# polarlightman/Scoring-rules-for-Gaussian-process-regression-a-new-approach-to-inference

Hardware: AMD Instinct MI355X
Metric: GP fit+predict+CRPS wall-clock (ms) at n=20k full / n=40k FITC; HBM GB/s & MFMA% (higher is better)
Workload: dtype f64; 1 GPU; C3 full GP fit(NLML+LOO-CRPS+LOO-LogS)+predict+score; n=20000, d=8, n_test=5000, kernel=ARD, parallelism=single

## Files before the change

### include/gpscore.h

```cpp
#ifndef GPSCORE_H
#define GPSCORE_H

#include <stdint.h>

#ifdef __cplusplus
extern "C" {
#endif

typedef struct gps_ctx gps_ctx;

enum { GPS_ARD = 0, GPS_RBF = 1 };
enum { GPS_FULL = 0, GPS_LOWER = 1 };

enum {
  GPS_OBJ_NLML = 0,
  GPS_OBJ_LOO_CRPS = 1,
  GPS_OBJ_LOO_LOGS = 2,
  GPS_OBJ_LOGDET = 3,
  GPS_OBJ_QUAD = 4,
  GPS_N_OBJ = 5
};
enum {
  GPS_SC_CRPS = 0, GPS_SC_LOGS = 1, GPS_SC_MSLL = 2, GPS_SC_SMSE = 3,
  GPS_SC_MSE = 4, GPS_SC_COVER = 5, GPS_N_SC = 6
// ... 7 lines not shown
const char* gps_last_error(gps_ctx* ctx);
int gps_ctx_set_stream(gps_ctx* ctx, void* hip_stream);
void* gps_ctx_stream(gps_ctx* ctx);
int gps_ctx_synchronize(gps_ctx* ctx);

enum {
  GPS_OPT_OVERLAP = 0,
  GPS_OPT_GEMM_MAP = 3,
  GPS_OPT_TINY_GEMM = 7,
  GPS_OPT_GRAM_REG = 9,
  GPS_OPT_GRAPH = 10,
  GPS_OPT_PRED_PRE = 11,
  GPS_OPT_DAG = 12,
  GPS_OPT_AR_CHUNKS = 15,
  GPS_OPT_DAG_TILES = 13,
  GPS_OPT_STREAM_K = 18,
  GPS_OPT_DAG_WGS = 19,
  GPS_OPT_DAG_GROUP = 17,
  GPS_OPT_SLAB_XCD = 26,
  GPS_OPT_DAG_ORDER = 25,
  GPS_OPT_FITC_DEP = 27,
  GPS_OPT_DAG_TILES_FULL = 28,
  GPS_OPT_DAG_KBATCH = 29,
};
int gps_ctx_set_option(gps_ctx* ctx, int key, int value);

enum { GPS_STAT_GRAPHS = 0, GPS_STAT_GRAPH_CAP = 1, GPS_STAT_GRAPH_OVERFLOW = 2,
       GPS_STAT_DEVICE_BYTES = 3, GPS_STAT_GRAPH_DROPPED = 4, GPS_STAT_GRAPH_EVICTED = 5,
       GPS_N_STATS = 6 };
int gps_ctx_stats(gps_ctx* ctx, int64_t* out, int cap);

int gps_dag_task_list(int T, int flags, uint32_t* out, int cap);
int gps_dag_task_list_ex(int T, int flags, int kb, int kg, uint32_t* out, int cap);

typedef struct gps_gemm_desc {
  int32_t lay_a, lay_b, epi;
  int32_t M, N, K;
  int64_t lda, ldb, ldc;
  double alpha, beta;
  int32_t tri, tri_off;
  int32_t lower_out, mirror;
  int32_t kend;
  int32_t tile, ksplit, map_mode;
  int32_t use_ws, sk_alone, dep_mode;
  int32_t reserved;
  int64_t ld_out, c_kslice_stride;
} gps_gemm_desc;
enum { GPS_GEMM_PLAN_TILE = 0, GPS_GEMM_PLAN_KSPLIT = 1, GPS_GEMM_PLAN_MAP = 2,
       GPS_GEMM_PLAN_SK_DP = 3, GPS_GEMM_PLAN_SK_WGS = 4, GPS_GEMM_PLAN_SLAB_XCD = 5,
       GPS_GEMM_PLAN_GRID_X = 6, GPS_GEMM_PLAN_GRID_Y = 7, GPS_N_GEMM_PLAN = 8 };
int gps_gemm_diag_check(const gps_gemm_desc* d, int have_c, int have_kscale, int have_w,
                        const int32_t* kr, int have_out0, int have_out1);
int gps_gemm_diag(gps_ctx* ctx, const gps_gemm_desc* d, const double* A, const double* B,
                  double* C, const double* kscale, const double* w, const int32_t* kr,
                  double* out0, double* out1, int32_t* plan);
int64_t gps_gemm_schedule(const gps_gemm_desc* d, const int32_t* kr, int have_kscale, int slots,
// ... 170 lines not shown
```

### scoring-rules-for-gaussian-process-regression-a-new-approach-to-inference_amd/csrc/api.hip

```cpp
#include "api_internal.h"

namespace gpsapi {

thread_local std::string g_err;

int fail(gps_ctx* ctx, int code, const std::string& msg) {
  if (ctx) ctx->err = msg;
  g_err = msg;
  return code;
}

hipError_t sync_ctx_streams(gps_ctx* ctx) {
  for (hipStream_t st : {ctx->stream, ctx->side, ctx->aux[0], ctx->aux[1]})
    if (st) {
      const hipError_t e = hipStreamSynchronize(st);
      if (e != hipSuccess) return e;
    }
  return hipSuccess;
}

hipError_t drop_graphs_in(gps_ctx* ctx, const void* p, size_t bytes) {
  if (!ctx || !p || ctx->pgraphs.empty()) return hipSuccess;
  const uintptr_t lo = (uintptr_t)p, hi = lo + bytes;
  bool synced = false;
// ... 192 lines not shown
  const int64_t np = ctx->fn_pad, mp = ctx->m_pad;
  GemmParams p = gp0();
  p.A = ctx->Knm.d(); p.lda = mp; p.B = Lx + c0 * mp; p.ldb = mp;
  p.M = (int)np; p.N = (int)(c1 - c0); p.K = (int)c1; p.tri = TRI_K_LE_J; p.tri_off = (int)c0;
  p.kend = (int)pad_to(ctx->m, 16);
  p.out0 = ctx->fslab.d() + (c0 / GPS_TILE) * np; p.ld_out = np;
  return gemm(ctx, LAY_N, LAY_T, EPI_ROWSQ, p, st);
}

int fitc_rowsq_dep(gps_ctx* ctx, const double* L, int* sig, int64_t ncols, int mode,
                   hipStream_t st, int64_t nb_dag) {
  const int64_t np = ctx->fn_pad, mp = ctx->m_pad;
  GemmParams p = gp0();
  p.A = ctx->Knm.d(); p.lda = mp; p.B = L; p.ldb = mp;
  p.M = (int)np; p.N = (int)ncols; p.K = (int)ncols; p.tri = TRI_K_LE_J;
  p.kend = (int)pad_to(ctx->m, 16);
  p.out0 = ctx->fslab.d(); p.ld_out = np;
  p.dep_sig = sig; p.dep_q = sig + kSigQueue; p.dep_err = static_cast<int*>(ctx->info.p) + 1;
  p.dep_grid = dag_width(ctx, nb_dag, true); p.dep_mode = mode;
  return gemm(ctx, LAY_N, LAY_T, EPI_ROWSQ, p, st);
}

int dag_list_key(const gps_ctx* ctx, int64_t nb) {
  return (int)(3 * nb + ctx->dag_order) << 8 | dag_kg(ctx, nb) << 4 | dag_kb(ctx, nb);
}
int dag_kb(const gps_ctx* ctx, int64_t nb) {
  if ((ctx->dag_kbatch & 256) && nb <= ctx->dag_tiles) return 1;
  return std::max(1, ctx->dag_kbatch & 15);
}
int dag_kg(const gps_ctx* ctx, int64_t nb) { return dag_kb(ctx, nb) > 1 ? ctx->dag_kbatch >> 4 & 3 : 0; }

bool dag_block(const gps_ctx* ctx, int64_t nb) {
  const int cap = ctx->dag_full && ctx->dag_tiles_full ? ctx->dag_tiles_full : ctx->dag_tiles;
  return ctx->dag && nb >= 2 && nb <= cap;
}

void dag_blocks(const gps_ctx* ctx, int64_t nb, std::vector<int>& sizes, int64_t& cnt) {
  if (nb <= 1) return;
  if (dag_block(ctx, nb)) {
    sizes.push_back((int)nb);
    cnt += dag_cnt_ints((int)nb);
    return;
  }
  dag_blocks(ctx, nb / 2, sizes, cnt);
  dag_blocks(ctx, nb - nb / 2, sizes, cnt);
}

int dag_width(const gps_ctx* ctx, int64_t nb, bool half) {
  const int auto_w = half ? std::max(4, ctx->ncu / 2) : ctx->ncu;
  return (int)std::min<int64_t>(ctx->dag_wgs > 0 ? ctx->dag_wgs : auto_w, std::max<int64_t>(4, 2 * nb * nb));
}

int potrf_inv_rec(gps_ctx* ctx, double* A, int64_t lda, double* Linv, int64_t ldl, double* W,
// ... 144 lines not shown
}


hipError_t zero_factor(gps_ctx* ctx, double* p, int64_t n_pad, hipStream_t s) {
  const hipError_t e = hipMemsetAsync(p, 0, (size_t)n_pad * n_pad * 8, s);
  if (e == hipSuccess) ctx->zeroed[(uintptr_t)p] = n_pad;
  return e;
}
bool factor_zeroed(const gps_ctx* ctx, const double* p, int64_t n_pad) {
  const auto it = ctx->zeroed.find((uintptr_t)p);
  return it != ctx->zeroed.end() && it->second == n_pad;
}

int potrf_inv(gps_ctx* ctx, double* A, int64_t n_pad, double* Linv, double* W, double* logdiag,
              int nreal, double* Lout) {
  if (!factor_zeroed(ctx, Linv, n_pad) || (Lout && !factor_zeroed(ctx, Lout, n_pad)))
    return fail(ctx, -1, "potrf_inv: factor buffer not zeroed for this size (internal contract)");
  std::vector<int> dsizes;
  int64_t dcnt = 0;
  dag_blocks(ctx, n_pad / GPS_TILE, dsizes, dcnt);
  for (int T : dsizes) {
    const int lk = dag_list_key(ctx, T);
    if (ctx->dag_lists.count(lk)) continue;
    const std::vector<uint32_t> tl = dag_task_list(T, ctx->dag_order, true, dag_kb(ctx, T), dag_kg(ctx, T));
    auto& e = ctx->dag_lists[lk];
    HIPCHK(ensure(ctx, e.first, tl.size() * 4));
    HIPCHK(hipMemcpyAsync(e.first.p, tl.data(), tl.size() * 4, hipMemcpyHostToDevice, ctx->stream));
    HIPCHK(hipStreamSynchronize(ctx->stream));
    e.second = (int)tl.size();
  }
  if (dcnt && ctx->dag_cnt.cap < (size_t)dcnt * 4) {
    HIPCHK(hipStreamSynchronize(ctx->stream));
    HIPCHK(ensure(ctx, ctx->dag_cnt, std::max<size_t>((size_t)dcnt * 4, (size_t)1 << 20)));
    HIPCHK(hipMemsetAsync(ctx->dag_cnt.p, 0, ctx->dag_cnt.cap, ctx->stream));
    HIPCHK(hipStreamSynchronize(ctx->stream));
  }
  auto eager = [&]() {
    ctx->sync_used = 0;
    ctx->pre.join = nullptr;
    ctx->dag_cnt_used = 0;
    ctx->fplan = gps_ctx::FactorPlan{};
    return potrf_inv_rec(ctx, A, n_pad, Linv, n_pad, W, (int)(n_pad / GPS_TILE), logdiag,
                         static_cast<int*>(ctx->info.p), 0, nreal, Lout, n_pad, true);
  };
  if (!ctx->graphs || ctx->prof || n_pad <= GPS_TILE) return eager();
  HIPCHK(ensure(ctx, ctx->ws_main, (size_t)kSplitWsDoubles * 8));
  HIPCHK(ensure(ctx, ctx->ws_side, (size_t)kSplitWsDoubles * 8));
  const bool pre = ctx->pre.kind == PRE_FITC_Q;
  std::vector<uintptr_t> key = {
      (uintptr_t)A, (uintptr_t)n_pad, (uintptr_t)Linv, (uintptr_t)W, (uintptr_t)logdiag,
      (uintptr_t)nreal, (uintptr_t)Lout, (uintptr_t)ctx->stream, (uintptr_t)ctx->side,
      (uintptr_t)ctx->overlap, (uintptr_t)ctx->gemm_map,
      (uintptr_t)g_tiny_gemm, (uintptr_t)g_stream_k, (uintptr_t)g_slab_xcd, (uintptr_t)ctx->info.p, (uintptr_t)ctx->ws_main.p,
      (uintptr_t)ctx->ws_side.p, (uintptr_t)pre,
      pre ? (uintptr_t)ctx->pre.n1 : 0, pre ? (uintptr_t)ctx->aux[0] : 0,
      pre ? (uintptr_t)ctx->Knm.p : 0, pre ? (uintptr_t)ctx->fslab.p : 0,
      pre ? (uintptr_t)ctx->fn_pad : 0, pre ? (uintptr_t)ctx->m_pad : 0, pre ? (uintptr_t)ctx->pre.sig : 0,
      (uintptr_t)ctx->dag, (uintptr_t)ctx->dag_tiles,
      (uintptr_t)(ctx->dag_full ? ctx->dag_tiles_full : 0), (uintptr_t)ctx->dag_kbatch, (uintptr_t)ctx->dag_group, (uintptr_t)ctx->dag_wgs, (uintptr_t)ctx->dag_half,
      (uintptr_t)ctx->dag_cnt.p, (uintptr_t)ctx->sk_cnt.p, (uintptr_t)ctx->dag_sig};
  for (int T : dsizes) key.push_back((uintptr_t)ctx->dag_lists[dag_list_key(ctx, T)].first.p);
  for (auto& g : ctx->pgraphs)
    if (g.key == key) {
      g.last_use = ++ctx->graph_tick;
      HIPCHK(hipGraphLaunch(g.exec, ctx->stream));
      ctx->fplan = g.plan;
      ctx->fplan.replayed = 1;
      return 0;
    }
  if (ctx->pgraphs.size() >= kMaxGraphs) {
    size_t lru = 0;
    for (size_t i = 1; i < ctx->pgraphs.size(); ++i)
      if (ctx->pgraphs[i].last_use < ctx->pgraphs[lru].last_use) lru = i;
    HIPCHK(sync_ctx_streams(ctx));
    const hipError_t e = hipGraphExecDestroy(ctx->pgraphs[lru].exec);
    ctx->pgraphs.erase(ctx->pgraphs.begin() + (ptrdiff_t)lru);
    ++ctx->graph_evicted;
    HIPCHK(e);
  }
  const size_t nev = 2 * (size_t)(n_pad / GPS_TILE) + 8;
  while (ctx->sync_ev.size() < nev) {
    hipEvent_t e;
// ... 218 lines not shown
      return 0;
    case GPS_OPT_FITC_DEP: ctx->fitc_dep = value != 0; return 0;
    case GPS_OPT_DAG_ORDER:
      ARGCHK(value >= 0 && value <= 2, "GPS_OPT_DAG_ORDER must be 0, 1 or 2");
      ctx->dag_order = value;
      return 0;
    case GPS_OPT_DAG_GROUP:
      ARGCHK(value >= 2 && value <= 4, "GPS_OPT_DAG_GROUP must be 2, 3 or 4");
      ctx->dag_group = value;
      return 0;
    case GPS_OPT_DAG_TILES:
      ARGCHK(value >= 2 && value <= 64, "GPS_OPT_DAG_TILES must be in 2..64");
      ctx->dag_tiles = value;
      return 0;
    case GPS_OPT_DAG_TILES_FULL:
      ARGCHK(value == 0 || (value >= 2 && value <= 64), "GPS_OPT_DAG_TILES_FULL must be 0 or in 2..64");
      ctx->dag_tiles_full = value;
      return 0;
    case GPS_OPT_DAG_KBATCH:
      ARGCHK(value >= 0 && (value & 15) <= 8 && (value >> 4 & 15) <= 3 && (value >> 9) == 0,
             "GPS_OPT_DAG_KBATCH must be B | g << 4 [| 256] with B in 0..8 and g in 0..3");
      ctx->dag_kbatch = (value & 15) < 2 ? 0 : value;
      return 0;
    default: return fail(ctx, -1, "unknown option");
  }
}

void* gps_ctx_stream(gps_ctx* ctx) { return ctx ? (void*)ctx->stream : nullptr; }

int gps_ctx_synchronize(gps_ctx* ctx) {
  if (int rc = bind(ctx)) return rc;
  HIPCHK(hipStreamSynchronize(ctx->stream));
  return 0;
}

int gps_ctx_stats(gps_ctx* ctx, int64_t* out, int cap) {
  if (int rc = bind(ctx)) return rc;
  ARGCHK(out != nullptr && cap >= 0, "out is NULL or cap < 0");
  size_t bytes = 0;
  for (DBuf* b : ctx_buffers(ctx)) bytes += b->cap;
  int64_t v[GPS_N_STATS];
  v[GPS_STAT_GRAPHS] = (int64_t)ctx->pgraphs.size();
  v[GPS_STAT_GRAPH_CAP] = (int64_t)kMaxGraphs;
  v[GPS_STAT_GRAPH_OVERFLOW] = ctx->graph_overflow;
  v[GPS_STAT_GRAPH_DROPPED] = ctx->graph_dropped;
  v[GPS_STAT_GRAPH_EVICTED] = ctx->graph_evicted;
  v[GPS_STAT_DEVICE_BYTES] = (int64_t)bytes;
  for (int i = 0; i < cap && i < GPS_N_STATS; ++i) out[i] = v[i];
  return GPS_N_STATS;
}

int gps_dag_task_list(int T, int flags, uint32_t* out, int cap) {
  return gps_dag_task_list_ex(T, flags, 1, 0, out, cap);
}

int gps_dag_task_list_ex(int T, int flags, int kb, int kg, uint32_t* out, int cap) {
  if (T < 2 || T > 64 || cap < 0 || (cap > 0 && !out) || (flags & ~13) || kb < 1 || kb > 8 || kg < 0 || kg > 3)
    return fail(nullptr, -1, "bad arguments");
  const std::vector<uint32_t> tl = dag_task_list(T, (flags >> 2 & 3) == 0 ? 1 : (flags >> 2 & 3) == 3 ? 0 : flags >> 2 & 3,
                                                 (flags & 1) != 0, kb, kg);
  for (int i = 0; i < cap && i < (int)tl.size(); ++i) out[i] = tl[i];
  return (int)tl.size();
}

int gps_phase_enable(gps_ctx* ctx, int on) {
  if (int rc = bind(ctx)) return rc;
  ctx->phase = on != 0;
  return 0;
}

int gps_phase_collect(gps_ctx* ctx, char* json_out, int64_t cap) {
  if (int rc = bind(ctx)) return rc;
  HIPCHK(sync_ctx_streams(ctx));
  std::map<std::string, std::pair<int, double>> agg;
  std::vector<std::string> order;
  for (size_t i = 1; i < ctx->ph_marks.size(); ++i) {
    const auto& m = ctx->ph_marks[i];
    if (m.first == "start") continue;
    float ms = 0.f;
    HIPCHK(hipEventElapsedTime(&ms, ctx->ph_ev[ctx->ph_marks[i - 1].second], ctx->ph_ev[m.second]));
    if (!agg.count(m.first)) order.push_back(m.first);
    agg[m.first].first += 1;
    agg[m.first].second += ms;
// ... 244 lines not shown
```

### scoring-rules-for-gaussian-process-regression-a-new-approach-to-inference_amd/csrc/api_internal.h

```cpp
#pragma once
#include <dlfcn.h>
#include <rccl/rccl.h>
#include <stdio.h>
#include <string.h>

#include <chrono>
#include <climits>
#include <cmath>
#include <condition_variable>
#include <map>
#include <memory>
#include <mutex>
#include <string>
#include <vector>

#include "gps_internal.h"
#include "gpscore.h"

using namespace gps;

namespace gpsapi {


struct DBuf {
// ... 60 lines not shown

struct gps_ctx {
  int device = 0;
  hipStream_t stream = nullptr;
  bool own_stream = true;
  hipStream_t side = nullptr;
  hipStream_t aux[2] = {nullptr, nullptr};
  bool overlap = true;
  int gemm_map = 0;
  int ar_chunks = 4;
  std::vector<hipEvent_t> ar_ev;
  int ncu = 0;
  std::vector<hipEvent_t> sync_ev;
  size_t sync_used = 0;
  bool graphs = true;
  bool pred_pre = true;
  bool dag = true;
  int dag_tiles = 20;
  int dag_group = 3;
  int dag_wgs = 0;
  int dag_order = 1;
  int dag_tiles_full = 40;
  int dag_kbatch = 8 | 256;
  bool dag_full = false;
  bool dag_half = false;
  bool fitc_dep = true;
  int* dag_sig = nullptr;
  DBuf dsig;
  std::map<int, std::pair<DBuf, int>> dag_lists;
  std::map<uintptr_t, int64_t> zeroed;
  DBuf dag_cnt;
  DBuf sk_cnt;
  int64_t dag_cnt_used = 0;
  struct PrePass {
    int kind = 0;
    int64_t n1 = 0;
    const double* L = nullptr;
    hipEvent_t join = nullptr;
    int* sig = nullptr;
  } pre;
  struct FactorPlan {
    int leaves = 0, dags = 0;
    int dag_tmin = 0, dag_tmax = 0;
    int gemms = 0, replayed = 0;
  } fplan;
  struct PotrfGraph {
// ... 124 lines not shown

hipError_t sync_ctx_streams(gps_ctx* ctx);
hipError_t drop_graphs_in(gps_ctx* ctx, const void* p, size_t bytes);
void forget_zeroed(gps_ctx* ctx, const void* p, size_t bytes);
hipError_t ensure(gps_ctx* ctx, DBuf& b, size_t bytes);
void release(gps_ctx* ctx, DBuf& b);
int get_event(gps_ctx* c);
int phase_event(gps_ctx* c, hipStream_t st);
void phase_mark(gps_ctx* c, const char* name);
hipEvent_t sync_event(gps_ctx* c);
GemmParams gp0();
const char* gemm_tag(int al, int bl, int epi, const GemmParams& p);
double gemm_flops(const GemmParams& p);
int gemm(gps_ctx* ctx, int al, int bl, int epi, const GemmParams& p, hipStream_t st = nullptr,
         GemmLaunchInfo* info = nullptr);
int gram(gps_ctx* ctx, const char* tag, const double* x, int n, const double* xp, int m, int d,
         const Theta& th, double diag_add, int lower, int pad_identity, double* out, int64_t ldo,
         int M, int N, hipStream_t st = nullptr);
int pred_rows(gps_ctx* ctx, int64_t r0, int64_t r1, const double* w, hipStream_t st);
int fitc_rowsq_cols(gps_ctx* ctx, const double* Lx, int64_t c0, int64_t c1, hipStream_t st);
int fitc_rowsq_dep(gps_ctx* ctx, const double* L, int* sig, int64_t ncols, int mode,
                   hipStream_t st, int64_t nb_dag);
int dag_list_key(const gps_ctx* ctx, int64_t nb);
int dag_kb(const gps_ctx* ctx, int64_t nb);
int dag_kg(const gps_ctx* ctx, int64_t nb);
bool dag_block(const gps_ctx* ctx, int64_t nb);
void dag_blocks(const gps_ctx* ctx, int64_t nb, std::vector<int>& sizes, int64_t& cnt);
int dag_width(const gps_ctx* ctx, int64_t nb, bool half);
int potrf_inv_rec(gps_ctx* ctx, double* A, int64_t lda, double* Linv, int64_t ldl, double* W,
                  int nb, double* logdiag, int* info, int base, int nreal, double* Lout,
                  int64_t ldlo, bool top = false);
size_t potrf_ws_doubles(int64_t n_pad);
int reset_info(gps_ctx* ctx);
hipError_t zero_factor(gps_ctx* ctx, double* p, int64_t n_pad, hipStream_t s);
bool factor_zeroed(const gps_ctx* ctx, const double* p, int64_t n_pad);
int potrf_inv(gps_ctx* ctx, double* A, int64_t n_pad, double* Linv, double* W, double* logdiag,
              int nreal, double* Lout);
int check_info(gps_ctx* ctx);
int set_theta(gps_ctx* ctx, Theta& th, int kind, const double* theta, int n_ell, int d);
int upload(gps_ctx* ctx, DBuf& b, const double* h, int64_t rows, int64_t cols, int64_t rows_pad);
void score_bundle(const double* sums, double nt, double out[GPS_N_SC]);
int bind(gps_ctx* ctx);
bool sharded(const gps_ctx* ctx);
std::vector<DBuf*> ctx_buffers(gps_ctx* ctx);
void leave_local_group(gps_ctx* ctx);
int group_barrier(gps_ctx* ctx, LocalGroup& G, size_t count);
// ... 26 lines not shown
```

### scoring-rules-for-gaussian-process-regression-a-new-approach-to-inference_amd/csrc/gps_internal.h

```cpp
#pragma once

#include <hip/hip_runtime.h>
#include <stdint.h>

#include <string>
#include <vector>

#define GPS_TILE 128
#define GPS_MAX_D 64

namespace gps {

inline int64_t pad_to(int64_t n, int64_t t = GPS_TILE) { return (n + t - 1) / t * t; }

struct GramParams {
  const double* x;
  const double* xp;
  double* out;
  int64_t ldo;
  int n, m;
  int M, N;
  int d;
  double sf2;
  double diag_add;
// ... 282 lines not shown
constexpr int kGemmItemInts = 8;
int64_t gemm_schedule(int alay, int blay, int epi, const GemmParams& p, GemmLaunchInfo& info,
                      int32_t* items, int64_t cap);

hipError_t launch_potrf_leaf(const double* A, int64_t lda, double* Linv, int64_t ldl,
                             double* Lout, int64_t ldlo, double* logdiag, int* info,
                             int base, int n_real_in_block, hipStream_t s);

struct DagParams {
  double* A; int64_t lda;
  double* Linv; int64_t ldl;
  double* Lout; int64_t ldlo;
  double* logdiag; int* info; int base; int nreal;
  int T;
  const uint32_t* tasks; int ntasks;
  int* cnt;
  unsigned long long spin_ticks;
  unsigned long long* trace = nullptr;
  int group = 3;
  int* sig = nullptr;
  int kbatch = 1;
};
hipError_t launch_potrf_dag(const DagParams& p, int nwg, hipStream_t s);
std::vector<uint32_t> dag_task_list(int T, int order = 1, bool fine = true, int kb = 1, int kg = 0);
inline int64_t dag_cnt_ints(int T) { return (16 + 2 * (int64_t)T * T + 63) / 64 * 64; }

hipError_t launch_gemv_lower(const double* L, int64_t ldl, const double* x, double* y,
                             int n_pad, hipStream_t s);
hipError_t launch_gemv_full(const double* M, int64_t ldm, const double* x, double* y,
                            int rows, int cols, hipStream_t s);
hipError_t launch_colred(const double* M, int64_t ldm, int rows, int cols, int lower,
                         const double* w, const double* rowscale, double* s1, double* s2,
                         double* slab, hipStream_t s, int crows = 256);
hipError_t launch_slab_sum(const double* slab, int64_t ld, int nslab, int64_t len,
                           const double* init, double* out, hipStream_t s);
hipError_t launch_sym_slab_sum(const double* slab, int64_t slice_stride, int nslab, int M,
                               const double* base, double* dst, hipStream_t s);

hipError_t launch_sym_pack(const double* slab, int64_t slice_stride, int nslab, int r0, int r1,
                           int M, double* packed, hipStream_t s);
hipError_t launch_sym_unpack(const double* packed, int m, int M, const double* base, int full,
                             double* dst, hipStream_t s);
hipError_t launch_full_loo(const double* y, const double* slab, int nslab, int64_t ld,
                           const double* beta, const double* logdiag, int n, double* alpha,
                           double* dinv, double* mu_loo, double* var_loo, double* obj,
                           double* part, hipStream_t s);
hipError_t launch_surface_point_sums(const double* y, const double* alpha, const double* dinv,
// ... 122 lines not shown
```

### scoring-rules-for-gaussian-process-regression-a-new-approach-to-inference_amd/csrc/kernels_potrf.hip

```cpp
#include <algorithm>
#include <queue>
#include <vector>

#include "gps_internal.h"

namespace gps {

namespace v4 {
typedef double d4 __attribute__((ext_vector_type(4)));
typedef double dv2 __attribute__((ext_vector_type(2)));
constexpr int TS = 17;
constexpr int TSZ = 16 * TS;
constexpr int NT = 36;
__device__ __forceinline__ constexpr int tix(int i, int j) { return i * (i + 1) / 2 + j; }

__device__ __forceinline__ double rl(double v, int lane) {
  const int lo = __builtin_amdgcn_readlane(__double2loint(v), lane);
  const int hi = __builtin_amdgcn_readlane(__double2hiint(v), lane);
  return __hiloint2double(hi, lo);
}
template <bool COH>
__device__ __forceinline__ void st_d(double* p, double v) {
  if constexpr (COH)
    __hip_atomic_store(reinterpret_cast<unsigned long long*>(p),
// ... 466 lines not shown
#pragma unroll
        for (int e = 0; e < 4; ++e)
#pragma unroll
          for (int j = 0; j < 2; ++j)
            cold[i][j][e] = ld64(rc, (uint32_t)(((int64_t)(16 * i + g + 4 * e) * s.ldc + 16 * j + r) * 8));
    }
    if (s.bt) wave_gemm32<true, G>(s.A, s.lda, s.B, s.ldb, s.kb, s.ke, acc);
    else wave_gemm32<false, G>(s.A, s.lda, s.B, s.ldb, s.kb, s.ke, acc);
  }
  __syncthreads();
  if (!s.active) return;
#pragma unroll
  for (int i = 0; i < 2; ++i)
#pragma unroll
    for (int e = 0; e < 4; ++e)
#pragma unroll
      for (int j = 0; j < 2; ++j) {
        double v = s.alpha * acc[i][j][e];
        if (s.beta != 0.0) v = fma(s.beta, cold[i][j][e], v);
        const int64_t row = 16 * i + g + 4 * e, col = 16 * j + r;
        st64(rc, (uint32_t)((row * s.ldc + col) * 8), v);
        if (s.C2) s.C2[row * s.ldc2 + col] = v;
      }
}

__device__ __forceinline__ void wave_gemm16(const double* Ap, int64_t lda, const double* B0,
                                            const double* B1, int64_t ldb, int ke0, int ke1,
                                            d4 (&acc)[2]) {
  const int lane = threadIdx.x & 63, r = lane & 15, g = lane >> 4;
  const __amdgpu_buffer_rsrc_t ra = rsrc(Ap, (uint32_t)(16 * lda * 8));
  const __amdgpu_buffer_rsrc_t rb0 = rsrc(B0, (uint32_t)(16 * ldb * 8));
  const __amdgpu_buffer_rsrc_t rb1 = rsrc(B1 ? B1 : B0, (uint32_t)(16 * ldb * 8));
  const int kmax = ke0 > ke1 ? ke0 : ke1;
  double a[8][4], b0[8][4], b1[8][4];
#pragma unroll
  for (int u = 0; u < 8; ++u) {
    const int k = 16 * u + 4 * g;
    const uint32_t o = (uint32_t)(((int64_t)r * lda + k) * 8), ob = (uint32_t)(((int64_t)r * ldb + k) * 8);
    if (16 * u < kmax) {
      const dv2 x0 = ld128(ra, o), x1 = ld128(ra, o + 16);
      a[u][0] = x0.x; a[u][1] = x0.y; a[u][2] = x1.x; a[u][3] = x1.y;
    }
    if (16 * u < ke0) {
      const dv2 x0 = ld128(rb0, ob), x1 = ld128(rb0, ob + 16);
      b0[u][0] = x0.x; b0[u][1] = x0.y; b0[u][2] = x1.x; b0[u][3] = x1.y;
    }
// ... 187 lines not shown
      f.C2 = nullptr;
      f.ldc2 = 0;
      if (type == 1) {
        const int64_t r0 = R + 16 * part;
        f.A = p.A + r0 * lda + K; f.lda = lda;
        f.B = p.Linv + K * ldl + K; f.ldb = ldl;
        f.C = p.A + r0 * lda + K; f.ldc = lda;
        if (p.Lout) { f.C2 = p.Lout + r0 * p.ldlo + K; f.ldc2 = p.ldlo; }
        f.alpha = 1.0; f.beta = 0.0;
        f.c0 = wave; f.c1 = 7 - wave; f.ke0 = 16 * (wave + 1); f.ke1 = 16 * (8 - wave);
        inc = U / NPF_TRSM;
        out = acnt + ti * T + tk;
      } else {
        const int64_t J = 128 * (int64_t)tj, rb = part >> 1, cb = 4 * (part & 1) + wave;
        f.A = p.A + (R + 16 * rb) * lda + K; f.lda = lda;
        f.B = p.A + J * lda + K; f.ldb = lda;
        f.C = p.A + (R + 16 * rb) * lda + J; f.ldc = lda;
        f.alpha = -1.0; f.beta = 1.0;
        f.c0 = (ti == tj && cb > rb) ? -1 : (int)cb; f.c1 = -1; f.ke0 = 128; f.ke1 = 0;
        inc = U / NPF_UPD;
        out = acnt + ti * T + tj;
      }
      run_fine(f);
    } else {
      inc = U / NP;
      Strip st;
      st.C2 = nullptr;
      st.ldc2 = 0;
      st.active = 1;
      const int64_t R = 128 * (int64_t)ti, q = 32 * part, wv = 32 * wave;
      switch (type) {
        case 1: {
          const int64_t K = 128 * (int64_t)tk;
          st.A = p.A + (R + q) * lda + K; st.lda = lda;
          st.B = p.Linv + (K + wv) * ldl + K; st.ldb = ldl; st.bt = 1;
          st.C = p.A + (R + q) * lda + K + wv; st.ldc = lda;
          if (p.Lout) { st.C2 = p.Lout + (R + q) * p.ldlo + K + wv; st.ldc2 = p.ldlo; }
          st.alpha = 1.0; st.beta = 0.0; st.kb = 0; st.ke = (int)wv + 32;
          out = acnt + ti * T + tk;
          break;
        }
        case 2: {
          const int64_t J = 128 * (int64_t)tj, K = 128 * (int64_t)tk;
          st.A = p.A + (R + q) * lda + K; st.lda = lda;
          st.B = p.A + (J + wv) * lda + K; st.ldb = lda; st.bt = 1;
          st.C = p.A + (R + q) * lda + J + wv; st.ldc = lda;
// ... 49 lines not shown
    }
    __syncthreads();
    const int n = 16 + 2 * T * T;
    for (int i = tid; i < n; i += 256)
      __hip_atomic_store(p.cnt + i, 0, __ATOMIC_RELAXED, __HIP_MEMORY_SCOPE_AGENT);
  }
}
}

hipError_t launch_potrf_dag(const DagParams& p, int nwg, hipStream_t s) {
  if ((p.lda & 1) || (p.ldl & 1) || (p.Lout && (p.ldlo & 1)) || p.T < 1 || p.T > 64 || nwg < 1 ||
      !p.tasks || !p.cnt || p.ntasks < 1 || p.kbatch < 1 || p.kbatch > 8)
    return hipErrorInvalidValue;
  if ((int64_t)128 * p.kbatch * std::max(p.lda, p.ldl) * 8 >= ((int64_t)1 << 31)) return hipErrorInvalidValue;
  auto k = p.trace ? (p.group == 2 ? dag::potrf_dag_kernel<true, 2>
                                    : p.group == 3 ? dag::potrf_dag_kernel<true, 3> : dag::potrf_dag_kernel<true, 4>)
                   : (p.group == 2 ? dag::potrf_dag_kernel<false, 2>
                                    : p.group == 3 ? dag::potrf_dag_kernel<false, 3> : dag::potrf_dag_kernel<false, 4>);
  if (p.group < 2 || p.group > 4) return hipErrorInvalidValue;
  hipLaunchKernelGGL(k, dim3(nwg), dim3(256), 0, s, p);
  return hipGetLastError();
}

double g_dag_weights[7] = {35.0, 6.0, 9.7, 11.7, 11.2, 9.3, 2.5};

std::vector<uint32_t> dag_task_list(int T, int order, bool fine, int kb, int kg) {
  struct Task { int type, i, j, k, len; std::vector<int> deps; double est = 0.0, rank = 0.0; };
  auto is_fine = [&](const Task& t) {
    return fine && ((t.type == 1 && t.i == t.k + 1) || (t.type == 2 && t.i == t.k + 1 && t.j == t.i));
  };
  auto batch_of = [&](int t, int nt, int keep, int& b0, int& b1) {
    const int nbat = kb > 1 ? std::max(0, nt - keep) : 0;
    if (t >= nbat) { b0 = t; b1 = t + 1; return; }
    b0 = t / kb * kb;
    b1 = std::min(b0 + kb, nbat);
  };
  std::vector<Task> tk;
  std::vector<int> leaf(T), xkk(T), trsm(T * T, -1), fin(T * T, -1);
  std::vector<int> upd_last(T * T, -1), updx_last(T * T, -1);
  auto add = [&](int type, int i, int j, int k, int len, std::vector<int> deps) {
    Task t;
    t.type = type; t.i = i; t.j = j; t.k = k; t.len = len;
    for (int d : deps)
      if (d >= 0) t.deps.push_back(d);
    tk.push_back(t);
    return (int)tk.size() - 1;
  };
  for (int k = 0; k < T; ++k) {
    leaf[k] = add(0, k, k, k, 1, {upd_last[k * T + k]});
    xkk[k] = leaf[k];
    for (int i = k + 1; i < T; ++i) trsm[i * T + k] = add(1, i, k, k, 1, {upd_last[i * T + k], xkk[k]});
    for (int j = k + 1; j < T; ++j)
      for (int i = j; i < T; ++i) {
        int b0, b1;
        batch_of(k, j, std::max(kg, fine && i == j ? 1 : 0), b0, b1);
        if (k != b1 - 1) continue;
        std::vector<int> deps = {upd_last[i * T + j]};
        for (int q = b0; q < b1; ++q) { deps.push_back(trsm[i * T + q]); deps.push_back(trsm[j * T + q]); }
        if (b1 - b0 == 1) deps = {trsm[i * T + k], trsm[j * T + k], upd_last[i * T + j]};
        upd_last[i * T + j] = add(2, i, j, b0, b1 - b0, deps);
      }
  }
  auto xfinal = [&](int j, int k) { return j == k ? xkk[k] : fin[j * T + k]; };
  for (int j = 0; j < T; ++j) {
    for (int k = 0; k < j; ++k)
      fin[j * T + k] = add(4, j, k, k, 1, {updx_last[j * T + k], xkk[j]});
    for (int i = j + 1; i < T; ++i)
      for (int k = 0; k <= j; ++k) {
        int b0, b1;
        batch_of(j - k, i - k, kg, b0, b1);
        if (j - k != b1 - 1) continue;
        std::vector<int> deps = {updx_last[i * T + k]};
        for (int q = b0 + k; q < b1 + k; ++q) { deps.push_back(trsm[i * T + q]); deps.push_back(xfinal(q, k)); }
        if (b1 - b0 == 1) deps = {trsm[i * T + j], xfinal(j, k), updx_last[i * T + k]};
        updx_last[i * T + k] = add(3, i, b0 + k, k, b1 - b0, deps);
      }
  }
  const int n = (int)tk.size();
  std::vector<std::vector<int>> succ(n);
  std::vector<int> indeg(n, 0);
  for (int t = 0; t < n; ++t)
    for (int d : tk[t].deps) { succ[d].push_back(t); ++indeg[t]; }
  if (order == 0) {
    auto dur = [&](const Task& t) { return t.type == 0 ? 36.0 : 4.0 * t.len; };
    for (int t = 0; t < n; ++t)
      for (int d : tk[t].deps) tk[t].est = std::max(tk[t].est, tk[d].est + dur(tk[d]) + 3.0);
  } else if (order == 2) {
    auto dur = [&](const Task& t) {
      return t.type == 0 ? 38.0 : is_fine(t) ? 4.0 : 9.0 * t.len;
    };
    for (int t = n - 1; t >= 0; --t) {
      double m = 0.0;
      for (int s2 : succ[t]) m = std::max(m, tk[s2].rank + 1.0);
      tk[t].rank = dur(tk[t]) + m;
      tk[t].est = -tk[t].rank;
    }
  } else {
    const double* w = g_dag_weights;
    auto dur = [&](const Task& t) {
      if (is_fine(t)) return w[1];
      switch (t.type) {
        case 0: return w[0];
        case 1: return w[2];
        case 2: return w[3] * t.len;
        case 3: return w[4] * t.len;
        default: return w[5];
      }
    };
    for (int t = n - 1; t >= 0; --t) {
      double m = 0.0;
      for (int s2 : succ[t]) m = std::max(m, tk[s2].rank + w[6]);
      tk[t].rank = dur(tk[t]) + m;
      tk[t].est = -tk[t].rank;
    }
  }
  std::priority_queue<std::pair<double, int>, std::vector<std::pair<double, int>>,
                      std::greater<std::pair<double, int>>> ready;
  for (int t = 0; t < n; ++t)
    if (!indeg[t]) ready.push({tk[t].est, t});
  std::vector<uint32_t> out;
  while (!ready.empty()) {
    const int t = ready.top().second;
    ready.pop();
    const Task& x = tk[t];
    const bool f = is_fine(x);
    const int parts = x.type == 0 ? 1 : !f ? dag::NP : x.type == 1 ? dag::NPF_TRSM : dag::NPF_UPD;
    for (int q = 0; q < parts; ++q)
      out.push_back((uint32_t)x.type | (uint32_t)q << 3 | (uint32_t)f << 7 | (uint32_t)x.i << 8 |
                    (uint32_t)((x.len - 1) & 3) << 14 | (uint32_t)x.j << 16 |
                    (uint32_t)((x.len - 1) >> 2) << 22 | (uint32_t)x.k << 24);
    for (int s2 : succ[t])
      if (!--indeg[s2]) ready.push({tk[s2].est, s2});
  }
  return out;
}

hipError_t launch_potrf_leaf(const double* A, int64_t lda, double* Linv, int64_t ldl, double* Lout,
                             int64_t ldlo, double* logdiag, int* info, int base, int nreal,
                             hipStream_t s) {
  if ((lda & 1) || (ldl & 1) || (Lout && (ldlo & 1))) return hipErrorInvalidValue;
  hipLaunchKernelGGL(v4::potrf_leaf_v4_kernel, dim3(1), dim3(256), 0, s, A, lda, Linv, ldl, Lout,
                     ldlo, logdiag, info, base, nreal);
  return hipGetLastError();
}

}
```

### scoring-rules-for-gaussian-process-regression-a-new-approach-to-inference_amd/gpscore/_lib.py

```python
from __future__ import annotations

import ctypes
import os

import numpy as np

_HERE = os.path.dirname(os.path.abspath(__file__))
LIB_PATH = os.environ.get("GPSCORE_LIB", os.path.join(_HERE, "libgpscore.so"))
ABI_VERSION = 900
GPS_N_STATS = 6
GPS_COMM_NONE, GPS_COMM_RCCL, GPS_COMM_LOCAL = 0, 1, 2
COMM_KINDS = {GPS_COMM_NONE: "none", GPS_COMM_RCCL: "rccl", GPS_COMM_LOCAL: "local"}

GPS_ARD, GPS_RBF = 0, 1
GPS_FULL, GPS_LOWER = 0, 1
GPS_OPT_OVERLAP, GPS_OPT_GEMM_MAP, GPS_OPT_TINY_GEMM, GPS_OPT_GRAM_REG = 0, 3, 7, 9
GPS_OPT_GRAPH = 10
GPS_OPT_PRED_PRE = 11
GPS_OPT_DAG = 12
GPS_OPT_DAG_TILES = 13
GPS_OPT_DAG_GROUP = 17
GPS_OPT_STREAM_K = 18
GPS_OPT_DAG_WGS = 19
GPS_OPT_DAG_ORDER = 25
GPS_OPT_SLAB_XCD = 26
GPS_OPT_FITC_DEP = 27
GPS_OPT_DAG_TILES_FULL = 28
GPS_OPT_DAG_KBATCH = 29
DAG_TILES_FULL_DEFAULT = 40
DAG_KBATCH_DEFAULT = 8 | 256
GPS_OPT_AR_CHUNKS = 15
OBJ_NAMES = ("nlml", "loo_crps", "loo_logs", "logdet", "quad")
SURFACE_NAMES = ("loo_crps", "insample_crps", "nlml", "loo_logs")
GPS_SURF_LOGS_ADD_NOISE = 1
GPS_BATCH_STALE_NOISE = 1
BATCH_MAX_N, BATCH_MAX_D = 128, 16
BATCH_FITC_MAX_M = 32
BATCH_FITC_TALL_MAX_N = 2048
BATCH_FULL_TALL_MAX_N = 512
SCORE_NAMES = ("test_crps", "test_logs", "test_msll", "test_smse", "test_mse", "test_cover")

_c_int, _c_i64, _c_dbl, _c_vp, _c_cp = (ctypes.c_int, ctypes.c_int64, ctypes.c_double,
                                        ctypes.c_void_p, ctypes.c_char_p)
_P = ctypes.POINTER(ctypes.c_double)

_PI = ctypes.POINTER(ctypes.c_int32)
_PI64 = ctypes.POINTER(ctypes.c_int64)
_PP = ctypes.POINTER(_P)


class GemmDesc(ctypes.Structure):
    _fields_ = [("lay_a", ctypes.c_int32), ("lay_b", ctypes.c_int32), ("epi", ctypes.c_int32),
                ("M", ctypes.c_int32), ("N", ctypes.c_int32), ("K", ctypes.c_int32),
# ... 5 lines not shown
                ("tile", ctypes.c_int32), ("ksplit", ctypes.c_int32), ("map_mode", ctypes.c_int32),
                ("use_ws", ctypes.c_int32), ("sk_alone", ctypes.c_int32),
                ("dep_mode", ctypes.c_int32), ("reserved", ctypes.c_int32),
                ("ld_out", _c_i64), ("c_kslice_stride", _c_i64)]


GEMM_PLAN_NAMES = ("tile", "ksplit", "map_mode", "sk_dp", "sk_wgs", "slab_xcd", "grid_x", "grid_y")
POTRF_PLAN_NAMES = ("n_pad", "leaves", "dags", "dag_tmin", "dag_tmax", "gemms", "replayed",
                    "reserved")

SIGNATURES = {
    "gps_version": (_c_int, []),
    "gps_build_id": (_c_int, [_c_cp, _c_int]),
    "gps_ctx_create": (_c_int, [_c_int, ctypes.POINTER(_c_vp)]),
    "gps_ctx_destroy": (_c_int, [_c_vp]),
    "gps_last_error": (_c_cp, [_c_vp]),
    "gps_ctx_set_stream": (_c_int, [_c_vp, _c_vp]),
    "gps_ctx_stream": (_c_vp, [_c_vp]),
    "gps_ctx_synchronize": (_c_int, [_c_vp]),
    "gps_ctx_set_option": (_c_int, [_c_vp, _c_int, _c_int]),
    "gps_ctx_stats": (_c_int, [_c_vp, _c_vp, _c_int]),
    "gps_dag_task_list": (_c_int, [_c_int, _c_int, _c_vp, _c_int]),
    "gps_dag_task_list_ex": (_c_int, [_c_int, _c_int, _c_int, _c_int, _c_vp, _c_int]),
    "gps_gemm_diag_check": (_c_int, [ctypes.POINTER(GemmDesc), _c_int, _c_int, _c_int, _PI, _c_int,
                                     _c_int]),
    "gps_gemm_schedule": (_c_i64, [ctypes.POINTER(GemmDesc), _PI, _c_int, _c_int, _PI, _PI, _c_i64]),
    "gps_gemm_diag": (_c_int, [_c_vp, ctypes.POINTER(GemmDesc), _P, _P, _P, _P, _P, _PI, _P, _P,
                               _PI]),
    "gps_potrf_diag": (_c_int, [_c_vp, _c_i64, _P, _c_i64, _P, _P, _P, _PI, _PI]),
    "gps_grad_terms_diag": (_c_int, [_c_vp, _c_int, _c_int, _c_i64, _c_i64, _c_i64, _c_dbl, _PP,
                                     _PP]),
    "gps_grad_contract_diag": (_c_int, [_c_vp, _c_i64, _c_int, _P, _P, _c_dbl, _P, _P, _c_i64, _P,
                                        _P, _P, _P]),
    "gps_fitc_contract_diag": (_c_int, [_c_vp, _c_i64, _c_i64, _c_i64, _c_int, _P, _P, _P, _c_dbl,
                                        _c_int, _PP, _PI64, _P, _PP, _P, _PP, _PP, _P, _P]),
    "gps_prof_enable": (_c_int, [_c_vp, _c_int]),
    "gps_prof_collect": (_c_int, [_c_vp, _c_cp, _c_i64]),
    "gps_phase_enable": (_c_int, [_c_vp, _c_int]),
    "gps_phase_collect": (_c_int, [_c_vp, _c_cp, _c_i64]),
    "gps_rccl_info": (_c_int, [ctypes.POINTER(_c_int), _c_cp, _c_int]),
    "gps_gram": (_c_int, [_c_vp, _c_int, _P, _c_i64, _P, _c_i64, _c_int, _c_dbl, _P, _c_int,
                          _c_dbl, _c_int, _P]),
    "gps_potrf": (_c_int, [_c_vp, _c_i64, _P, _c_i64, _P]),
    "gps_potrs": (_c_int, [_c_vp, _c_i64, _c_i64, _P, _c_i64, _P, _c_i64, _P, _c_i64]),
    "gps_diag_inv": (_c_int, [_c_vp, _c_i64, _P, _c_i64, _P]),
    "gps_gemm": (_c_int, [_c_vp, _c_int, _c_int, _c_i64, _c_i64, _c_i64, _c_dbl, _P, _c_i64, _P,
# ... 338 lines not shown
```

Baseline: 8.262 fit+predict+score units/s (C3 full GP, whole job).

## Add whole-tile MFMA task form for long update tasks in the potrf DAG

Adds a 'tile form' for type-2 (SYRK/GEMM update) and type-3 (inverse update) tasks in the DAG Cholesky/inverse. Tasks long enough and far enough from the critical diagonal are now run as a single work item, with each wave computing a 64x64 block through a triple-buffered f64 MFMA loop. Previously these tasks were split into NP strip parts. The scheduler's cost model weights tile tasks differently and the task encoding gains a bit for the form. It is on by default (minlen 2, distance 2) and aims to cut per-strip overhead and raise MFMA reuse, at the risk of coarser load balance and longer serial tasks.

```diff
diff --git a/include/gpscore.h b/include/gpscore.h
--- a/include/gpscore.h
+++ b/include/gpscore.h
@@ -53,6 +53,7 @@
   GPS_OPT_FITC_DEP = 27,
   GPS_OPT_DAG_TILES_FULL = 28,
   GPS_OPT_DAG_KBATCH = 29,
+  GPS_OPT_DAG_TILE_FORM = 30,
 };
 int gps_ctx_set_option(gps_ctx* ctx, int key, int value);
 
@@ -63,6 +64,7 @@
 
 int gps_dag_task_list(int T, int flags, uint32_t* out, int cap);
 int gps_dag_task_list_ex(int T, int flags, int kb, int kg, uint32_t* out, int cap);
+int gps_dag_task_list_tf(int T, int flags, int kb, int kg, int tf, uint32_t* out, int cap);
 
 typedef struct gps_gemm_desc {
   int32_t lay_a, lay_b, epi;
diff --git a/scoring-rules-for-gaussian-process-regression-a-new-approach-to-inference_amd/csrc/api.hip b/scoring-rules-for-gaussian-process-regression-a-new-approach-to-inference_amd/csrc/api.hip
--- a/scoring-rules-for-gaussian-process-regression-a-new-approach-to-inference_amd/csrc/api.hip
+++ b/scoring-rules-for-gaussian-process-regression-a-new-approach-to-inference_amd/csrc/api.hip
@@ -238,13 +238,14 @@
 }
 
 int dag_list_key(const gps_ctx* ctx, int64_t nb) {
-  return (int)(3 * nb + ctx->dag_order) << 8 | dag_kg(ctx, nb) << 4 | dag_kb(ctx, nb);
+  return ((int)(3 * nb + ctx->dag_order) << 8 | dag_kg(ctx, nb) << 4 | dag_kb(ctx, nb)) << 8 | dag_tf(ctx, nb);
 }
 int dag_kb(const gps_ctx* ctx, int64_t nb) {
   if ((ctx->dag_kbatch & 256) && nb <= ctx->dag_tiles) return 1;
   return std::max(1, ctx->dag_kbatch & 15);
 }
 int dag_kg(const gps_ctx* ctx, int64_t nb) { return dag_kb(ctx, nb) > 1 ? ctx->dag_kbatch >> 4 & 3 : 0; }
+int dag_tf(const gps_ctx* ctx, int64_t nb) { return dag_kb(ctx, nb) > 1 ? ctx->dag_tile_form : 0; }
 
 bool dag_block(const gps_ctx* ctx, int64_t nb) {
   const int cap = ctx->dag_full && ctx->dag_tiles_full ? ctx->dag_tiles_full : ctx->dag_tiles;
@@ -435,7 +436,7 @@
   for (int T : dsizes) {
     const int lk = dag_list_key(ctx, T);
     if (ctx->dag_lists.count(lk)) continue;
-    const std::vector<uint32_t> tl = dag_task_list(T, ctx->dag_order, true, dag_kb(ctx, T), dag_kg(ctx, T));
+    const std::vector<uint32_t> tl = dag_task_list(T, ctx->dag_order, true, dag_kb(ctx, T), dag_kg(ctx, T), dag_tf(ctx, T));
     auto& e = ctx->dag_lists[lk];
     HIPCHK(ensure(ctx, e.first, tl.size() * 4));
     HIPCHK(hipMemcpyAsync(e.first.p, tl.data(), tl.size() * 4, hipMemcpyHostToDevice, ctx->stream));
@@ -470,7 +471,7 @@
       pre ? (uintptr_t)ctx->Knm.p : 0, pre ? (uintptr_t)ctx->fslab.p : 0,
       pre ? (uintptr_t)ctx->fn_pad : 0, pre ? (uintptr_t)ctx->m_pad : 0, pre ? (uintptr_t)ctx->pre.sig : 0,
       (uintptr_t)ctx->dag, (uintptr_t)ctx->dag_tiles,
-      (uintptr_t)(ctx->dag_full ? ctx->dag_tiles_full : 0), (uintptr_t)ctx->dag_kbatch, (uintptr_t)ctx->dag_group, (uintptr_t)ctx->dag_wgs, (uintptr_t)ctx->dag_half,
+      (uintptr_t)(ctx->dag_full ? ctx->dag_tiles_full : 0), (uintptr_t)ctx->dag_kbatch, (uintptr_t)ctx->dag_tile_form, (uintptr_t)ctx->dag_group, (uintptr_t)ctx->dag_wgs, (uintptr_t)ctx->dag_half,
       (uintptr_t)ctx->dag_cnt.p, (uintptr_t)ctx->sk_cnt.p, (uintptr_t)ctx->dag_sig};
   for (int T : dsizes) key.push_back((uintptr_t)ctx->dag_lists[dag_list_key(ctx, T)].first.p);
   for (auto& g : ctx->pgraphs)
@@ -735,6 +736,11 @@
              "GPS_OPT_DAG_KBATCH must be B | g << 4 [| 256] with B in 0..8 and g in 0..3");
       ctx->dag_kbatch = (value & 15) < 2 ? 0 : value;
       return 0;
+    case GPS_OPT_DAG_TILE_FORM:
+      ARGCHK(value >= 0 && (value & 15) <= 8 && (value >> 8) == 0 && ((value & 15) || !value),
+             "GPS_OPT_DAG_TILE_FORM must be 0 or minlen | d << 4 with minlen in 1..8 and d in 0..15");
+      ctx->dag_tile_form = value;
+      return 0;
     default: return fail(ctx, -1, "unknown option");
   }
 }
@@ -768,10 +774,15 @@
 }
 
 int gps_dag_task_list_ex(int T, int flags, int kb, int kg, uint32_t* out, int cap) {
-  if (T < 2 || T > 64 || cap < 0 || (cap > 0 && !out) || (flags & ~13) || kb < 1 || kb > 8 || kg < 0 || kg > 3)
+  return gps_dag_task_list_tf(T, flags, kb, kg, 0, out, cap);
+}
+
+int gps_dag_task_list_tf(int T, int flags, int kb, int kg, int tf, uint32_t* out, int cap) {
+  if (T < 2 || T > 64 || cap < 0 || (cap > 0 && !out) || (flags & ~13) || kb < 1 || kb > 8 || kg < 0 || kg > 3 ||
+      tf < 0 || (tf >> 8) || (tf & 15) > 8 || (tf && !(tf & 15)))
     return fail(nullptr, -1, "bad arguments");
   const std::vector<uint32_t> tl = dag_task_list(T, (flags >> 2 & 3) == 0 ? 1 : (flags >> 2 & 3) == 3 ? 0 : flags >> 2 & 3,
-                                                 (flags & 1) != 0, kb, kg);
+                                                 (flags & 1) != 0, kb, kg, tf);
   for (int i = 0; i < cap && i < (int)tl.size(); ++i) out[i] = tl[i];
   return (int)tl.size();
 }
diff --git a/scoring-rules-for-gaussian-process-regression-a-new-approach-to-inference_amd/csrc/api_internal.h b/scoring-rules-for-gaussian-process-regression-a-new-approach-to-inference_amd/csrc/api_internal.h
--- a/scoring-rules-for-gaussian-process-regression-a-new-approach-to-inference_amd/csrc/api_internal.h
+++ b/scoring-rules-for-gaussian-process-regression-a-new-approach-to-inference_amd/csrc/api_internal.h
@@ -106,6 +106,7 @@
   int dag_order = 1;
   int dag_tiles_full = 40;
   int dag_kbatch = 8 | 256;
+  int dag_tile_form = 2 | 2 << 4;
   bool dag_full = false;
   bool dag_half = false;
   bool fitc_dep = true;
@@ -276,6 +277,7 @@
 int fitc_rowsq_dep(gps_ctx* ctx, const double* L, int* sig, int64_t ncols, int mode,
                    hipStream_t st, int64_t nb_dag);
 int dag_list_key(const gps_ctx* ctx, int64_t nb);
+int dag_tf(const gps_ctx* ctx, int64_t nb);
 int dag_kb(const gps_ctx* ctx, int64_t nb);
 int dag_kg(const gps_ctx* ctx, int64_t nb);
 bool dag_block(const gps_ctx* ctx, int64_t nb);
diff --git a/scoring-rules-for-gaussian-process-regression-a-new-approach-to-inference_amd/csrc/gps_internal.h b/scoring-rules-for-gaussian-process-regression-a-new-approach-to-inference_amd/csrc/gps_internal.h
--- a/scoring-rules-for-gaussian-process-regression-a-new-approach-to-inference_amd/csrc/gps_internal.h
+++ b/scoring-rules-for-gaussian-process-regression-a-new-approach-to-inference_amd/csrc/gps_internal.h
@@ -328,7 +328,8 @@
   int kbatch = 1;
 };
 hipError_t launch_potrf_dag(const DagParams& p, int nwg, hipStream_t s);
-std::vector<uint32_t> dag_task_list(int T, int order = 1, bool fine = true, int kb = 1, int kg = 0);
+std::vector<uint32_t> dag_task_list(int T, int order = 1, bool fine = true, int kb = 1, int kg = 0,
+                                    int tf = 0);
 inline int64_t dag_cnt_ints(int T) { return (16 + 2 * (int64_t)T * T + 63) / 64 * 64; }
 
 hipError_t launch_gemv_lower(const double* L, int64_t ldl, const double* x, double* y,
diff --git a/scoring-rules-for-gaussian-process-regression-a-new-approach-to-inference_amd/csrc/kernels_potrf.hip b/scoring-rules-for-gaussian-process-regression-a-new-approach-to-inference_amd/csrc/kernels_potrf.hip
--- a/scoring-rules-for-gaussian-process-regression-a-new-approach-to-inference_amd/csrc/kernels_potrf.hip
+++ b/scoring-rules-for-gaussian-process-regression-a-new-approach-to-inference_amd/csrc/kernels_potrf.hip
@@ -512,6 +512,109 @@
         st64(rc, (uint32_t)((row * s.ldc + col) * 8), v);
         if (s.C2) s.C2[row * s.ldc2 + col] = v;
       }
+}
+
+template <bool BT>
+__device__ __forceinline__ void wave_gemm64(const double* Ap, int64_t lda, const double* Bp,
+                                            int64_t ldb, int kb, int ke, d4 (&acc)[4][4]) {
+  const int lane = threadIdx.x & 63, r = lane & 15, g = lane >> 4;
+  const __amdgpu_buffer_rsrc_t ra = rsrc(Ap, (uint32_t)(64 * lda * 8));
+  const __amdgpu_buffer_rsrc_t rb = rsrc(Bp, (uint32_t)((BT ? 64 : ke > 128 ? ke : 128) * ldb * 8));
+  struct Frag { double a[4][4], b[4][4]; };
+  const int nc = (ke - kb) / 16;
+  const uint32_t oa0 = (uint32_t)(((int64_t)r * lda + kb + 4 * g) * 8), sa = (uint32_t)(16 * lda * 8);
+  const uint32_t ob0 = BT ? (uint32_t)(((int64_t)r * ldb + kb + 4 * g) * 8)
+                          : (uint32_t)(((int64_t)(kb + 4 * g) * ldb + r) * 8);
+  const uint32_t sb = BT ? (uint32_t)(16 * ldb * 8) : (uint32_t)(ldb * 8);
+  auto load = [&](int c, Frag& f) {
+    const uint32_t oa = oa0 + 128u * (uint32_t)c;
+#pragma unroll
+    for (int i = 0; i < 4; ++i) {
+      const dv2 a0 = ld128(ra, oa + i * sa), a1 = ld128(ra, oa + i * sa + 16);
+      f.a[i][0] = a0.x; f.a[i][1] = a0.y; f.a[i][2] = a1.x; f.a[i][3] = a1.y;
+    }
+    if constexpr (BT) {
+      const uint32_t ob = ob0 + 128u * (uint32_t)c;
+#pragma unroll
+      for (int i = 0; i < 4; ++i) {
+        const dv2 b0 = ld128(rb, ob + i * sb), b1 = ld128(rb, ob + i * sb + 16);
+        f.b[i][0] = b0.x; f.b[i][1] = b0.y; f.b[i][2] = b1.x; f.b[i][3] = b1.y;
+      }
+    } else {
+      const uint32_t ob = ob0 + 16u * (uint32_t)c * sb;
+#pragma unroll
+      for (int e = 0; e < 4; ++e)
+#pragma unroll
+        for (int i = 0; i < 4; ++i) f.b[i][e] = ld64(rb, ob + e * sb + 128u * i);
+    }
+  };
+  auto mma = [&](const Frag& f) {
+#pragma unroll
+    for (int kk = 0; kk < 4; ++kk)
+#pragma unroll
+      for (int i = 0; i < 4; ++i)
+#pragma unroll
+        for (int j = 0; j < 4; ++j)
+          acc[i][j] = __builtin_amdgcn_mfma_f64_16x16x4f64(f.a[i][kk], f.b[j][kk], acc[i][j], 0, 0, 0);
+  };
+  Frag f0, f1, f2;
+  load(0, f0);
+  load(1, f1);
+  int c = 0;
+  for (; c + 5 <= nc; c += 3) {
+    load(c + 2, f2);
+    mma(f0);
+    load(c + 3, f0);
+    mma(f1);
+    load(c + 4, f1);
+    mma(f2);
+  }
+  const int rem = nc - c;
+  if (rem >= 3) load(c + 2, f2);
+  mma(f0);
+  if (rem == 4) load(c + 3, f0);
+  mma(f1);
+  if (rem >= 3) mma(f2);
+  if (rem == 4) mma(f0);
+}
+
+struct Tile {
+  const double* A; int64_t lda;
+  const double* B; int64_t ldb; int bt;
+  double* C; int64_t ldc;
+  double alpha, beta;
+  int kb, ke;
+};
+
+__device__ __forceinline__ void run_tile(const Tile& s) {
+  const int lane = threadIdx.x & 63, r = lane & 15, g = lane >> 4;
+  const __amdgpu_buffer_rsrc_t rc = rsrc(s.C, (uint32_t)(64 * s.ldc * 8));
+  d4 acc[4][4];
+#pragma unroll
+  for (int i = 0; i < 4; ++i)
+#pragma unroll
+    for (int j = 0; j < 4; ++j) acc[i][j] = (d4){0.0, 0.0, 0.0, 0.0};
+  if (s.bt) wave_gemm64<true>(s.A, s.lda, s.B, s.ldb, s.kb, s.ke, acc);
+  else wave_gemm64<false>(s.A, s.lda, s.B, s.ldb, s.kb, s.ke, acc);
+  const uint32_t oc = (uint32_t)(((int64_t)g * s.ldc + r) * 8), sc = (uint32_t)(4 * s.ldc * 8);
+#pragma unroll
+  for (int i = 0; i < 4; ++i) {
+    double cold[4][4];
+    if (s.beta != 0.0) {
+#pragma unroll
+      for (int e = 0; e < 4; ++e)
+#pragma unroll
+        for (int j = 0; j < 4; ++j) cold[j][e] = ld64(rc, oc + (4 * i + e) * sc + 128u * j);
+    }
+#pragma unroll
+    for (int e = 0; e < 4; ++e)
+#pragma unroll
+      for (int j = 0; j < 4; ++j) {
+        double v = s.alpha * acc[i][j][e];
+        if (s.beta != 0.0) v = fma(s.beta, cold[j][e], v);
+        st64(rc, oc + (4 * i + e) * sc + 128u * j, v);
+      }
+  }
 }
 
 __device__ __forceinline__ void wave_gemm16(const double* Ap, int64_t lda, const double* B0,
@@ -745,6 +848,27 @@
         out = acnt + ti * T + tj;
       }
       run_fine(f);
+    } else if (w >> 23 & 1) {
+      Tile tl;
+      const int64_t R = 128 * (int64_t)ti + 64 * (wave >> 1), J = 128 * (int64_t)tj,
+                    K = 128 * (int64_t)tk, wc = 64 * (wave & 1);
+      if (type == 2) {
+        tl.A = p.A + R * lda + K; tl.lda = lda;
+        tl.B = p.A + (J + wc) * lda + K; tl.ldb = lda; tl.bt = 1;
+        tl.C = p.A + R * lda + J + wc; tl.ldc = lda;
+        tl.alpha = -1.0; tl.beta = 1.0; tl.kb = 0;
+        out = acnt + ti * T + tj;
+      } else {
+        tl.A = p.A + R * lda + J; tl.lda = lda;
+        tl.B = p.Linv + J * ldl + K + wc; tl.ldb = ldl; tl.bt = 0;
+        tl.C = p.Linv + R * ldl + K + wc; tl.ldc = ldl;
+        tl.alpha = 1.0; tl.beta = tj == tk ? 0.0 : 1.0;
+        tl.kb = tj == tk ? (int)wc : 0;
+        out = xcnt + ti * T + tk;
+      }
+      tl.ke = 128 * len;
+      inc = len * U;
+      run_tile(tl);
     } else {
       inc = U / NP;
       Strip st;
@@ -840,10 +964,15 @@
   return hipGetLastError();
 }
 
-double g_dag_weights[7] = {35.0, 6.0, 9.7, 11.7, 11.2, 9.3, 2.5};
-
-std::vector<uint32_t> dag_task_list(int T, int order, bool fine, int kb, int kg) {
-  struct Task { int type, i, j, k, len; std::vector<int> deps; double est = 0.0, rank = 0.0; };
+double g_dag_weights[8] = {35.0, 6.0, 9.7, 11.7, 11.2, 9.3, 2.5, 2.0};
+
+std::vector<uint32_t> dag_task_list(int T, int order, bool fine, int kb, int kg, int tf) {
+  struct Task { int type, i, j, k, len; std::vector<int> deps; double est = 0.0, rank = 0.0; int tile = 0; };
+  const int tf_min = tf & 15, tf_d = tf >> 4 & 15;
+  auto tile_form = [&](const Task& t) {
+    if (!tf_min || (t.type != 2 && t.type != 3) || t.len < tf_min) return false;
+    return t.type == 2 ? t.i > t.j && t.j - (t.k + t.len) >= tf_d : t.i - (t.j + t.len) >= tf_d;
+  };
   auto is_fine = [&](const Task& t) {
     return fine && ((t.type == 1 && t.i == t.k + 1) || (t.type == 2 && t.i == t.k + 1 && t.j == t.i));
   };
@@ -859,6 +988,7 @@
   auto add = [&](int type, int i, int j, int k, int len, std::vector<int> deps) {
     Task t;
     t.type = type; t.i = i; t.j = j; t.k = k; t.len = len;
+    t.tile = tile_form(t);
     for (int d : deps)
       if (d >= 0) t.deps.push_back(d);
     tk.push_back(t);
@@ -900,12 +1030,12 @@
   for (int t = 0; t < n; ++t)
     for (int d : tk[t].deps) { succ[d].push_back(t); ++indeg[t]; }
   if (order == 0) {
-    auto dur = [&](const Task& t) { return t.type == 0 ? 36.0 : 4.0 * t.len; };
+    auto dur = [&](const Task& t) { return t.type == 0 ? 36.0 : 4.0 * t.len * (t.tile ? 2.0 : 1.0); };
     for (int t = 0; t < n; ++t)
       for (int d : tk[t].deps) tk[t].est = std::max(tk[t].est, tk[d].est + dur(tk[d]) + 3.0);
   } else if (order == 2) {
     auto dur = [&](const Task& t) {
-      return t.type == 0 ? 38.0 : is_fine(t) ? 4.0 : 9.0 * t.len;
+      return t.type == 0 ? 38.0 : is_fine(t) ? 4.0 : 9.0 * t.len * (t.tile ? 2.0 : 1.0);
     };
     for (int t = n - 1; t >= 0; --t) {
       double m = 0.0;
@@ -917,11 +1047,12 @@
     const double* w = g_dag_weights;
     auto dur = [&](const Task& t) {
       if (is_fine(t)) return w[1];
+      const double tw = t.tile ? w[7] : 1.0;
       switch (t.type) {
         case 0: return w[0];
         case 1: return w[2];
-        case 2: return w[3] * t.len;
-        case 3: return w[4] * t.len;
+        case 2: return w[3] * t.len * tw;
+        case 3: return w[4] * t.len * tw;
         default: return w[5];
       }
     };
@@ -942,11 +1073,11 @@
     ready.pop();
     const Task& x = tk[t];
     const bool f = is_fine(x);
-    const int parts = x.type == 0 ? 1 : !f ? dag::NP : x.type == 1 ? dag::NPF_TRSM : dag::NPF_UPD;
+    const int parts = x.type == 0 || x.tile ? 1 : !f ? dag::NP : x.type == 1 ? dag::NPF_TRSM : dag::NPF_UPD;
     for (int q = 0; q < parts; ++q)
       out.push_back((uint32_t)x.type | (uint32_t)q << 3 | (uint32_t)f << 7 | (uint32_t)x.i << 8 |
                     (uint32_t)((x.len - 1) & 3) << 14 | (uint32_t)x.j << 16 |
-                    (uint32_t)((x.len - 1) >> 2) << 22 | (uint32_t)x.k << 24);
+                    (uint32_t)((x.len - 1) >> 2) << 22 | (uint32_t)x.tile << 23 | (uint32_t)x.k << 24);
     for (int s2 : succ[t])
       if (!--indeg[s2]) ready.push({tk[s2].est, s2});
   }
diff --git a/scoring-rules-for-gaussian-process-regression-a-new-approach-to-inference_amd/gpscore/_lib.py b/scoring-rules-for-gaussian-process-regression-a-new-approach-to-inference_amd/gpscore/_lib.py
--- a/scoring-rules-for-gaussian-process-regression-a-new-approach-to-inference_amd/gpscore/_lib.py
+++ b/scoring-rules-for-gaussian-process-regression-a-new-approach-to-inference_amd/gpscore/_lib.py
@@ -27,8 +27,10 @@
 GPS_OPT_FITC_DEP = 27
 GPS_OPT_DAG_TILES_FULL = 28
 GPS_OPT_DAG_KBATCH = 29
+GPS_OPT_DAG_TILE_FORM = 30
 DAG_TILES_FULL_DEFAULT = 40
 DAG_KBATCH_DEFAULT = 8 | 256
+DAG_TILE_FORM_DEFAULT = 2 | 2 << 4
 GPS_OPT_AR_CHUNKS = 15
 OBJ_NAMES = ("nlml", "loo_crps", "loo_logs", "logdet", "quad")
 SURFACE_NAMES = ("loo_crps", "insample_crps", "nlml", "loo_logs")
@@ -80,6 +82,7 @@
     "gps_ctx_stats": (_c_int, [_c_vp, _c_vp, _c_int]),
     "gps_dag_task_list": (_c_int, [_c_int, _c_int, _c_vp, _c_int]),
     "gps_dag_task_list_ex": (_c_int, [_c_int, _c_int, _c_int, _c_int, _c_vp, _c_int]),
+    "gps_dag_task_list_tf": (_c_int, [_c_int, _c_int, _c_int, _c_int, _c_int, _c_vp, _c_int]),
     "gps_gemm_diag_check": (_c_int, [ctypes.POINTER(GemmDesc), _c_int, _c_int, _c_int, _PI, _c_int,
                                      _c_int]),
     "gps_gemm_schedule": (_c_i64, [ctypes.POINTER(GemmDesc), _PI, _c_int, _c_int, _PI, _PI, _c_i64]),
```

New measurement: 8.374 fit+predict+score units/s (C3 full GP, whole job) (median of 6 runs). +1.4%, better.
